# zhuduowang/Change3D

Hardware: AMD Instinct MI355X
Metric: train images/sec (256x256 pairs, X3D-L BCD) (higher is better)
Workload: dtype bf16; 1 GPU; BCD X3D-L bf16, B=32/GPU, 256x256 synthetic LEVIR-CD-shaped pairs, T=3, train step (fwd+BCE/Dice+bwd+Adam); global_batch=32, parallelism=dp1, dist_world_size=1, hip_graph=False, full=False, settle_steps=40, input=resident in HBM

## Files before the change

### change3d_amd/_lib.py

```python
import ctypes as C
import os

_HERE = os.path.dirname(os.path.abspath(__file__))
LIB_PATH = os.environ.get("C3D_LIB") or os.path.join(_HERE, "lib", "libchange3d_hip.so")

DT_F32, DT_BF16 = 0, 1
PRO_NONE, PRO_BN_SE_SWISH, PRO_AFFINE2 = 0, 1, 2
EPI_STORE, EPI_STATS, EPI_SWISH_SE_BWD, EPI_ADD = 0, 1, 2, 3
AUG_NONE, AUG_BCD, AUG_SCD, AUG_BDA = 0, 1, 2, 3
ROWS_DENSE, ROWS_FRAME, ROWS_STRIDE2, ROWS_S2SHIFT = 0, 1, 2, 3
SC_NONE, SC_IDENTITY, SC_BN, SC_RAW = 0, 1, 2, 3
STAT_STRIPES = 16
OPT_SIDE_STREAM, OPT_STEM_MFMA, OPT_CONVT_MFMA, OPT_FUSE_WGRAD, OPT_FOLD_SE, OPT_MASK_IN_DGRAD, OPT_DW_RING, OPT_PW_WGRAD_V2, OPT_DW_FWD_HV, OPT_PW_CFWD, OPT_PW_CDG, OPT_DW_T4 = 0, 1, 2, 3, 4, 5, 6, 7, 8, 9, 10, 11
STAGE_SEPARATE_FINALIZE, STAGE_NO_WEIGHT_IMAGES, STAGE_SEPARATE_RESIDUAL, STAGE_SEPARATE_WGRAD = 1, 2, 4, 8

vp, i32, i64, f32, f64 = C.c_void_p, C.c_int32, C.c_int64, C.c_float, C.c_double


class BnFin(C.Structure):
    _fields_ = [("ticket", vp), ("gamma", vp), ("beta", vp), ("running_mean", vp), ("running_var", vp), ("nbt", vp),
                ("ss", vp), ("mr", vp), ("count", f64), ("momentum", f32), ("eps", f32), ("training", i32),
                ("batch", i32), ("sums", vp)]


class PwArgs(C.Structure):
    _fields_ = [("x", vp), ("x2", vp), ("y", vp), ("e1", vp), ("w", vp), ("pro_p", vp), ("pro_gate", vp),
                ("epi_p", vp), ("epi_gate", vp), ("epi_q", vp), ("stats", vp),
                ("M", i64), ("gstride", i64), ("rows_per_sample", i64),
# ... 85 lines not shown
    "c3d_block_out_fwd_fin": (i32, [vp, C.POINTER(BnFin), vp, C.POINTER(BnFin), i32, vp, i64, i32, i32, i32, vp]),
    "c3d_block_out_bwd": (i32, [vp, vp, vp, vp, vp, vp, vp, vp, vp, i64, i32, i32, i32, vp]),
    "c3d_block_out_bwd_fin": (i32, [vp, vp, vp, vp, vp, vp, vp, vp, vp, i64, i32, i32, i32, C.POINTER(BnFin),
                                    C.POINTER(BnFin), vp]),
    "c3d_frame_absdiff": (i32, [vp, vp, i32, i32, i64, i32, i32, i32, i32, vp]),
    "c3d_enhance_apply": (i32, [vp, vp, vp, i32, i32, i64, i32, i32, i32, vp]),
    "c3d_enhance_bwd_mask": (i32, [vp, vp, vp, i32, i32, i64, i32, i32, i32, vp]),
    "c3d_enhance_bwd_apply": (i32, [vp, vp, vp, vp, i32, i32, i64, i32, i32, i32, i32, vp]),
    "c3d_stem_enhance_fwd": (i32, [vp, vp, vp, vp, i32, i32, i64, i32, i32, i32, i32, i32, vp]),
    "c3d_stem_enhance_mid": (i32, [vp, vp, vp, vp, i32, i32, i64, i32, i32, i32, vp]),
    "c3d_stem_enhance_bwd": (i32, [vp, vp, vp, vp, vp, vp, vp, i32, i32, i64, i32, i32, i32, i32, i32, vp]),
    "c3d_frame_scatter": (i32, [vp, vp, i32, i32, i64, i32, i32, i32, i32, vp]),
    "c3d_stem_fwd": (i32, [vp, vp, vp, vp, vp, i32, i32, i32, i32, i32, vp]),
    "c3d_stem_bwd_dv": (i32, [vp, vp, vp, vp, vp, vp, vp, vp, i32, i32, i32, i32, i32, vp]),
    "c3d_stem_bwd_wx": (i32, [vp, vp, vp, vp, vp, i32, i32, i32, i32, i32, i32, i32, i32, vp]),
    "c3d_convT4s2_fwd": (i32, [vp, vp, vp, vp, i64, vp, i32, i32, i32, i32, i32, vp]),
    "c3d_convT4s2_bwd_data": (i32, [vp, vp, vp, i32, i32, i32, i32, i32, vp]),
    "c3d_convT4s2_wgrad_ws_floats": (i64, [i32, i32, i32, i32]),
    "c3d_convT4s2_wgrad": (i32, [vp, vp, vp, vp, i32, i32, i32, i32, i32, vp]),
    "c3d_col_sum": (i32, [vp, vp, i64, i32, i32, i32, vp]),
    "c3d_head3x3_fwd": (i32, [vp, vp, vp, i32, i32, i32, i32, i32, i32, i32, vp]),
    "c3d_head3x3_bwd_ws_floats": (i64, [i32, i32, i32, i32]),
    "c3d_head3x3_bwd": (i32, [vp, vp, vp, vp, vp, vp, vp, i32, i32, i32, i32, i32, i32, i32, vp]),
    "c3d_bce_dice_fwd": (i32, [vp, vp, i64, vp, vp, vp]),
    "c3d_bce_dice_bwd": (i32, [vp, vp, vp, vp, i64, vp, vp]),
    "c3d_ce2d_fwd": (i32, [vp, vp, i64, i32, i64, i64, i64, i64, vp, vp, vp]),
    "c3d_ce2d_bwd": (i32, [vp, vp, vp, vp, i64, i32, i64, i64, i64, i64, vp, vp]),
    "c3d_cossim_fwd": (i32, [vp, vp, vp, i64, i32, i64, i64, i64, i64, i64, vp, vp, vp]),
    "c3d_cossim_bwd": (i32, [vp, vp, vp, vp, i64, i32, i64, i64, i64, i64, i64, vp, vp, vp]),
    "c3d_adam_step": (i32, [vp, vp, vp, vp, i64, vp, f32, f32, f32, f32, f32, f32, f32, vp]),
# ... 95 lines not shown
```

### change3d_amd/csrc/launch_hints.h

```cpp
#pragma once
#include <cstdint>
#include <hip/hip_runtime.h>
#include "../../include/change3d_hip.h"

extern thread_local int c3d_side_launch;

extern int c3d_option_stem_mfma;
extern int c3d_option_convt_mfma;
extern int c3d_option_dw_ring;
extern int c3d_option_pw_wgrad_v2;
extern int c3d_option_dw_fwd_hv;
extern int c3d_option_pw_cfwd;
extern int c3d_option_pw_cdg;
extern int c3d_option_dw_t4;
#pragma GCC visibility push(hidden)
extern int c3d_option_side_stream;
extern int c3d_option_fuse_wgrad;
extern int c3d_option_fold_se;
extern int c3d_option_mask_in_dgrad;
extern int c3d_option_wgrad_chain;
#pragma GCC visibility pop
bool c3d_detail_pw_cdg_a_shape(int Kp, int Np, int64_t M);
bool c3d_detail_pw_cdg_c_shape(int Kp, int Np, int64_t M, int64_t rows_per_sample);
bool c3d_detail_pw_cdg_a_accepts(const c3d_pw_args* args);
bool c3d_detail_pw_cdg_c_accepts(const c3d_pw_args* args);
int c3d_detail_pw_cdg_a(const c3d_pw_args* args, int* parts_out, void* stream);
int c3d_detail_pw_cdg_c(const c3d_pw_args* args, int* parts_out, void* stream);
int c3d_detail_pw_wgrad_reduce(const float* ws, float* dw, int N, int K, int parts, int sn, int sk, hipStream_t stream);
void c3d_detail_pw_wgrad_v2_forget(const float* ws);
// ... 1 lines not shown
```

### change3d_amd/csrc/options.hip

```cpp
#include "../../include/change3d_hip.h"
#include "common.h"
#include "launch_hints.h"
#include <cstring>
#include <cxxabi.h>

namespace {
enum Norm {
  BOOL,
  CLAMP,
  MASK,
  BIT_OFF,
};
}

#define C3D_OPTIONS(X)                                                    \
  X(C3D_OPT_SIDE_STREAM, c3d_option_side_stream, BOOL, 0, 1)              \
  X(C3D_OPT_STEM_MFMA, c3d_option_stem_mfma, CLAMP, 2, 2)                 \
  X(C3D_OPT_CONVT_MFMA, c3d_option_convt_mfma, BOOL, 0, 1)                \
  X(C3D_OPT_FUSE_WGRAD, c3d_option_fuse_wgrad, MASK, 3, 3)                \
  X(C3D_OPT_FOLD_SE, c3d_option_fold_se, BOOL, 0, 1)                      \
  X(C3D_OPT_MASK_IN_DGRAD, c3d_option_mask_in_dgrad, MASK, 3, 3)          \
  X(C3D_OPT_DW_RING, c3d_option_dw_ring, MASK, 15, 13)                    \
  X(C3D_OPT_PW_WGRAD_V2, c3d_option_pw_wgrad_v2, MASK, 1, 1)              \
  X(C3D_OPT_PW_WGRAD_V2, c3d_option_wgrad_chain, BIT_OFF, 2, 1)           \
  X(C3D_OPT_DW_FWD_HV, c3d_option_dw_fwd_hv, MASK, 7, 5)                  \
  X(C3D_OPT_PW_CFWD, c3d_option_pw_cfwd, MASK, 3, 3)                      \
  X(C3D_OPT_PW_CDG, c3d_option_pw_cdg, MASK, 3, 3)                        \
  X(C3D_OPT_DW_T4, c3d_option_dw_t4, BOOL, 0, 1)

#define X(id, var, how, arg, dflt) int var = dflt;
C3D_OPTIONS(X)
#undef X

extern "C" int c3d_set_option(int32_t option, int32_t value) {
  static const struct { int32_t id; int* var; Norm how; int arg; } rows[] = {
#define X(id, var, how, arg, dflt) {id, &var, how, arg},
      C3D_OPTIONS(X)
#undef X
  };
  int rc = C3D_E_BADARG;
  for (const auto& r : rows) {
    if (r.id != option) continue;
    switch (r.how) {
// ... 35 lines not shown
```

### change3d_amd/csrc/stem.hip

```cpp
#include "common.h"
#include "stem_mfma.h"
#include <cstdlib>
#include "../../include/change3d_hip.h"

namespace {

constexpr int ST_C = 24;
constexpr int ST_CI = 3;
constexpr int ST_TH = 8, ST_TW = 16;
constexpr int ST_MAXT = 5;

template <typename T> struct RawS;
template <> struct RawS<bf16_t> {
  typedef uint4 type;
  static __device__ __forceinline__ type load(const bf16_t* p) { return *reinterpret_cast<const uint4*>(p); }
  static __device__ __forceinline__ void cvt(const type& v, float (&f)[8]) {
    f[0] = __uint_as_float(v.x << 16); f[1] = __uint_as_float(v.x & 0xffff0000u);
    f[2] = __uint_as_float(v.y << 16); f[3] = __uint_as_float(v.y & 0xffff0000u);
    f[4] = __uint_as_float(v.z << 16); f[5] = __uint_as_float(v.z & 0xffff0000u);
    f[6] = __uint_as_float(v.w << 16); f[7] = __uint_as_float(v.w & 0xffff0000u);
  }
};
template <> struct RawS<float> {
  struct type { float4 a, b; };
// ... 449 lines not shown
  const int ntiles = ((W + ST_TW - 1) / ST_TW) * ((H + ST_TH - 1) / ST_TH);
  int bsplit = (2 * 256 + ntiles - 1) / ntiles;
  if (bsplit > B) bsplit = B;
  if (bsplit < 1) bsplit = 1;
  const int tpw = 1;
  dim3 grid(ntiles, bsplit);
  hipStream_t s = reinterpret_cast<hipStream_t>(stream);
  if (dtype == C3D_DT_F32)
    return c3d_launch_lds<stem_bwd_wx_kernel<float>>(grid, SW_THREADS, lds, s, x, w_t, (const float*)dv, dw_t, dP, g, t_first,
                                                     n_frames, per_sample, tpw);
  if (dtype == C3D_DT_BF16)
    return c3d_launch_lds<stem_bwd_wx_kernel<bf16_t>>(grid, SW_THREADS, lds, s, x, w_t, (const bf16_t*)dv, dw_t, dP, g, t_first,
                                                      n_frames, per_sample, tpw);
  return C3D_E_BADARG;
}
```

### change3d_amd/csrc/stem_mfma.h

```cpp
#pragma once
#include <hip/hip_runtime.h>

bool c3d_stem_mfma_enabled();
int c3d_stem_fwd_mfma(const float* x, const float* w_t, const float* w_xy, void* u, double* sums, int B, int T, int H,
                      int W, int dtype, hipStream_t s);
int c3d_stem_bwd_dv_mfma(const float* x, const float* w_t, const float* w_xy, const void* g0, const void* u,
                         const float* coef, void* dv, float* dw_xy, int B, int T, int H, int W, int dtype, hipStream_t s);
int c3d_stem_bwd_wx_mfma(const float* x, const float* w_t, const void* dv, float* dw_t, float* dP, int B, int T, int H,
                         int W, int t_first, int n_frames, int per_sample, int dtype, hipStream_t s);
```

### change3d_amd/csrc/stem_mfma.hip

```cpp
#include "common.h"
#include "stem_mfma.h"
#include "launch_hints.h"
#include <cstdlib>
#include "../../include/change3d_hip.h"

namespace {

constexpr int SC = 24, SCI = 3;
constexpr int TH = 8, TW = 32;
constexpr int IH = TH + 2, IW = TW + 2;
constexpr int IHW = IH * IW;
constexpr int NTHR = 256;
constexpr int KS = 7;

struct Geom { int B, T, H, W; };

__device__ __forceinline__ f32x4_t mfma4(float a, float b, f32x4_t c) {
  return __builtin_amdgcn_mfma_f32_16x16x4f32(a, b, c, 0, 0, 0);
}

template <int TT> struct XTile {
  static constexpr int ITEMS = SCI * TT * IHW;
  static constexpr int NL = (ITEMS + NTHR - 1) / NTHR;
  float r[NL];
// ... 627 lines not shown
      if (tap < 9 && ci < SCI) {
#pragma unroll
        for (int i = 0; i < 4; ++i) wred[(wave * 32 + mt * 16 + 4 * g4 + i) * 32 + ci * 9 + tap] = dwacc[mt][nt][i];
      }
    }
  __syncthreads();
  for (int i = tid; i < SC * 27; i += NTHR) {
    const int c = i / 27, k = i - c * 27;
    float a = 0.f;
#pragma unroll
    for (int w = 0; w < 4; ++w) a += wred[(w * 32 + c) * 32 + k];
    atomicAdd(dw_t + (size_t)c * 27 + k, a);
  }
}

template <typename T, int TT>
int fwd_t(const float* x, const float* w_t, const float* w_xy, void* u, double* sums, const Geom& g, hipStream_t s) {
  const size_t lds = (2 * 4 * 2 * 32 + (size_t)SCI * TT * IHW) * sizeof(float);
  const int ntiles = ((g.W + TW - 1) / TW) * ((g.H + TH - 1) / TH);
  static const int env_tpw = c3d_env("C3D_STEM_FWD_TPW") ? atoi(c3d_env("C3D_STEM_FWD_TPW")) : 0;
  int tpw = 8;
  while (tpw > 1 && (long)((ntiles + tpw - 1) / tpw) * g.B < 1024) tpw >>= 1;
  if (env_tpw > 0) tpw = env_tpw;
  dim3 grid((ntiles + tpw - 1) / tpw, g.B);
  stem_fwd_mfma_kernel<T, TT><<<grid, NTHR, lds, s>>>(x, w_t, w_xy, reinterpret_cast<T*>(u), sums, g, tpw);
  return 0;
}

template <typename T, int TT>
int dv_t(const float* x, const float* w_t, const float* w_xy, const void* g0, const void* u, const float* coef, void* dv,
// ... 21 lines not shown
  if (lds > 160 * 1024) return C3D_E_UNSUPPORTED;
  const int ntiles = ((g.W + TW - 1) / TW) * ((g.H + TH - 1) / TH);
  int bsplit = (2 * 256 + ntiles - 1) / ntiles;
  if (bsplit > g.B) bsplit = g.B;
  if (bsplit < 1) bsplit = 1;
  if (sizeof(T) == 2 && c3d_option_stem_mfma >= 2 && (!dP || n_frames <= (TT - 2 > 0 ? TT - 2 : 1))) {
    size_t lb = ((size_t)TT * IHW * SC + 8 + (size_t)TT * IHW * 4 + 8) * sizeof(bf16_t);
    if (lb < 4 * 32 * 32 * sizeof(float)) lb = 4 * 32 * 32 * sizeof(float);
    return c3d_launch_lds<stem_bwd_wx_bf16_kernel<TT>>(dim3(ntiles, bsplit), NTHR, lb, s, x, w_t, reinterpret_cast<const bf16_t*>(dv),
                                                       dw_t, dP, g, t_first, n_frames, per_sample);
  }
  return c3d_launch_lds<stem_bwd_wx_mfma_kernel<T, TT>>(dim3(ntiles, bsplit), NTHR, lds, s, x, w_t, reinterpret_cast<const T*>(dv),
                                                        dw_t, dP, g, t_first, n_frames, per_sample);
}

#define STEM_DISPATCH(FN, ...)                                                         \
  if (dtype == C3D_DT_F32) {                                                           \
    if (T == 3) return FN<float, 3>(__VA_ARGS__);                                      \
    if (T == 4) return FN<float, 4>(__VA_ARGS__);                                      \
    if (T == 5) return FN<float, 5>(__VA_ARGS__);                                      \
  } else if (dtype == C3D_DT_BF16) {                                                   \
    if (T == 3) return FN<bf16_t, 3>(__VA_ARGS__);                                     \
    if (T == 4) return FN<bf16_t, 4>(__VA_ARGS__);                                     \
    if (T == 5) return FN<bf16_t, 5>(__VA_ARGS__);                                     \
  }                                                                                    \
  return C3D_E_UNSUPPORTED;

}

bool c3d_stem_mfma_enabled() { return c3d_option_stem_mfma != 0; }
// ... 3 lines not shown
  const Geom g{B, T, H, W};
  STEM_DISPATCH(fwd_t, x, w_t, w_xy, u, sums, g, s)
}

int c3d_stem_bwd_dv_mfma(const float* x, const float* w_t, const float* w_xy, const void* g0, const void* u,
                         const float* coef, void* dv, float* dw_xy, int B, int T, int H, int W, int dtype, hipStream_t s) {
  const Geom g{B, T, H, W};
  STEM_DISPATCH(dv_t, x, w_t, w_xy, g0, u, coef, dv, dw_xy, g, s)
}

int c3d_stem_bwd_wx_mfma(const float* x, const float* w_t, const void* dv, float* dw_t, float* dP, int B, int T, int H,
                         int W, int t_first, int n_frames, int per_sample, int dtype, hipStream_t s) {
  const Geom g{B, T, H, W};
  STEM_DISPATCH(wx_t, x, w_t, dv, dw_t, dP, g, t_first, n_frames, per_sample, s)
}
```

### change3d_amd/model/x3d.py

```python
import math

import os

import torch
import torch.nn as nn

from .. import ops
from ..ops import cpad

BN_EPS, BN_MOM = 1e-5, 0.1


def round_width(width, multiplier, min_width=8, divisor=8, ceil=False):
    if not multiplier:
        return width
    width *= multiplier
    min_width = min_width or divisor
    if ceil:
        out = max(min_width, int(math.ceil(width / divisor)) * divisor)
    else:
        out = max(min_width, int(width + divisor / 2) // divisor * divisor)
    if out < 0.9 * width:
        out += divisor
    return int(out)
# ... 56 lines not shown
    g = torch.empty_like(u)
    dsums = torch.zeros(2 * C, dtype=torch.float64, device=dev)
    ops.block_out_bwd(dyc, y, u, None, g, mr, None, dsums, None, M, C, dt)
    return _stem_backward_convs(ctx, xin, u, mr, g, dsums, frames_grad)


def _stem_backward_convs(ctx, xin, u, mr, g, dsums, frames_grad=None):
    stem = ctx.stem
    B, _, T, H, W = xin.shape
    dev, dt = xin.device, ops.dt_code(stem.act_dtype)
    conv_s, conv_t = stem.conv.conv_t, stem.conv.conv_xy
    C = conv_s.weight.shape[0]
    M = B * T * H * W
    coef = _f32(3 * cpad(C), dev)
    ops.bn_bwd_coef(dsums, M, stem.norm, mr, C, coef)
    dv = torch.empty_like(u)
    ops.stem_bwd_dv(xin, conv_s.weight, conv_t.weight, g, u, coef, dv, ops.grad_of(conv_t.weight), B, T, H, W, dt)
    dx = None
    if frames_grad is not None:
        gp, t0, nf = frames_grad
        ops.stem_bwd_wx(xin, conv_s.weight, dv, ops.grad_of(conv_s.weight), gp, B, T, H, W, t0, nf, False, dt)
    elif ctx.x_needs_grad:
        t0, nf = stem.grad_frames if stem.grad_frames is not None else (0, T)
        dx = torch.zeros_like(xin)
        ops.stem_bwd_wx(xin, conv_s.weight, dv, ops.grad_of(conv_s.weight), dx, B, T, H, W, t0, nf, True, dt)
    else:
        ops.stem_bwd_wx(xin, conv_s.weight, dv, ops.grad_of(conv_s.weight), None, B, T, H, W, 0, 0, False, dt)
    return dx


def _assemble_clip(ctx, pre, post, frames):
    ops.require_gpu(pre, "encoder input")
    B, Ci, H, W = pre.shape
    K = frames.shape[2]
    if Ci != 3 or tuple(frames.shape) != (1, 3, K, H, W) or tuple(post.shape) != tuple(pre.shape):
        raise NotImplementedError("clip assembly expects (B,3,H,W) images and (1,3,K,H,W) perception frames")
    clip = torch.empty((B, 3, K + 2, H, W), dtype=torch.float32, device=pre.device)
    ops.build_clip(pre.detach().contiguous().float(), post.detach().contiguous().float(),
                   frames.detach().contiguous().float(), clip, B, K, H, W)
    ctx.frames, ctx.K, ctx.x_needs_grad = frames, K, False
    ctx.need_frames = ctx.needs_input_grad[2]
    return clip

# ... 355 lines not shown
```

### change3d_amd/ops.py

```python
import ctypes as C

import os

import torch

from . import _lib as L
from ._lib import (OPT_CONVT_MFMA, OPT_DW_FWD_HV, OPT_DW_RING, OPT_DW_T4, OPT_FOLD_SE, OPT_FUSE_WGRAD, OPT_MASK_IN_DGRAD, OPT_PW_CDG, OPT_PW_CFWD, OPT_PW_WGRAD_V2, OPT_SIDE_STREAM, OPT_STEM_MFMA, STAGE_NO_WEIGHT_IMAGES, STAGE_SEPARATE_FINALIZE,
                   STAGE_SEPARATE_RESIDUAL, STAGE_SEPARATE_WGRAD)
from ._lib import (DT_BF16, DT_F32, EPI_ADD, EPI_STATS, EPI_STORE, EPI_SWISH_SE_BWD, PRO_AFFINE2,
                   PRO_BN_SE_SWISH, PRO_NONE, ROWS_DENSE, ROWS_FRAME, ROWS_S2SHIFT, ROWS_STRIDE2, SC_BN,
                   SC_IDENTITY, SC_NONE, SC_RAW, STAT_STRIPES)


def cpad(c):
    return (c + 7) // 8 * 8


def dt_code(dtype):
    if dtype == torch.float32:
        return DT_F32
    if dtype == torch.bfloat16:
        return DT_BF16
    raise TypeError(f"unsupported activation dtype {dtype} (float32 | bfloat16)")

# ... 76 lines not shown

def weights_version():
    return _weights_version[0]


def bump_weights_version():
    _weights_version[0] += 1


SIDE_STREAM = os.environ.get("C3D_WGRAD_SIDE", "1") != "0"
_side_streams = {}
_side_pending = []
_side_state = {"seq": 0}


def set_option(option, value):
    L.check(L.lib().c3d_set_option(int(option), int(value)), "c3d_set_option")


def last_kernel():
    return L.lib().c3d_last_kernel().decode()


def launch_count():
    return int(L.lib().c3d_launch_count())


def side_run(fn, *tensors):
    in_backward = False
    if SIDE_STREAM:
        try:
            torch.autograd.Variable._execution_engine.queue_callback(side_join)
# ... 303 lines not shown
            t_dst, 1 if accumulate else 0, dtype, _stream())


def stem_fwd(x, w_t, w_xy, u, sums, B, T, H, W, dtype):
    _launch("c3d_stem_fwd", x.numel() * 4 + u.numel() * _es(dtype), L.lib().c3d_stem_fwd, _p(x), _p(w_t), _p(w_xy), _p(u), _p(sums), B, T, H, W, dtype, _stream())


def stem_bwd_dv(x, w_t, w_xy, g0, u, coef, dv, dw_xy, B, T, H, W, dtype):
    _launch("c3d_stem_bwd_dv", x.numel() * 4 + 3 * u.numel() * _es(dtype), L.lib().c3d_stem_bwd_dv, _p(x), _p(w_t), _p(w_xy), _p(g0), _p(u), _p(coef), _p(dv), _p(dw_xy), B, T, H,
                                    W, dtype, _stream())


def stem_bwd_wx(x, w_t, dv, dw_t, dP, B, T, H, W, t_first, n_frames, per_sample, dtype):
    _launch("c3d_stem_bwd_wx", x.numel() * 4 + dv.numel() * _es(dtype), L.lib().c3d_stem_bwd_wx, _p(x), _p(w_t), _p(dv), _p(dw_t), _p(dP), B, T, H, W, t_first, n_frames,
                                    1 if per_sample else 0, dtype, _stream())


def convT_fwd(inp, w, bias, skip_ptr, skip_bstride, out, B, h, wd, C_, dtype):
    _launch("c3d_convT4s2_fwd", (inp.numel() + 2 * out.numel()) * _es(dtype), L.lib().c3d_convT4s2_fwd, _p(inp), _p(w), _p(bias), skip_ptr, skip_bstride, _p(out), B, h, wd, C_,
                                     dtype, _stream())


def convT_bwd_data(dout, w, din, B, h, wd, C_, dtype):
    _launch("c3d_convT4s2_bwd_data", (dout.numel() + din.numel()) * _es(dtype), L.lib().c3d_convT4s2_bwd_data, _p(dout), _p(w), _p(din), B, h, wd, C_, dtype, _stream())


CONVT_MFMA = os.environ.get("C3D_CONVT_MFMA", "1") != "0"


def convT_wgrad(t, dout, dw, B, h, wd, C_, dtype):
# ... 373 lines not shown
```

### include/change3d_hip.h

```cpp
#ifndef CHANGE3D_HIP_H
#define CHANGE3D_HIP_H
#include <stdint.h>

#ifdef __cplusplus
extern "C" {
#endif

#define C3D_DT_F32 0
#define C3D_DT_BF16 1

#define C3D_E_BADARG (-1)
#define C3D_E_UNSUPPORTED (-2)

int c3d_abi_version(void);
const char* c3d_build_info(void);
int c3d_device_cus(void);

#define C3D_PRO_NONE 0
#define C3D_PRO_BN_SE_SWISH 1
#define C3D_PRO_AFFINE2 2

#define C3D_EPI_STORE 0
#define C3D_EPI_STATS 1
#define C3D_STAT_STRIPES 16
// ... 161 lines not shown
                         int32_t Cp, int32_t t_mid, int32_t dtype, void* stream);
int c3d_stem_enhance_bwd(const void* dout, const void* u, const float* ss, const void* dd, const float* mr, void* g,
                         double* dsums, int32_t B, int32_t T, int64_t HW, int32_t C, int32_t Cp, int32_t t_pre,
                         int32_t t_post, int32_t dtype, void* stream);
int c3d_frame_scatter(const void* src, void* dst, int32_t B, int32_t T, int64_t HW, int32_t Cp,
                      int32_t t_dst, int32_t accumulate, int32_t dtype, void* stream);

int c3d_stem_fwd(const float* x, const float* w_t, const float* w_xy, void* u, double* sums, int32_t B,
                 int32_t T, int32_t H, int32_t W, int32_t dtype, void* stream);
int c3d_stem_bwd_dv(const float* x, const float* w_t, const float* w_xy, const void* g0, const void* u,
                    const float* coef, void* dv, float* dw_xy, int32_t B, int32_t T, int32_t H, int32_t W,
                    int32_t dtype, void* stream);
int c3d_stem_bwd_wx(const float* x, const float* w_t, const void* dv, float* dw_t, float* dP, int32_t B,
                    int32_t T, int32_t H, int32_t W, int32_t t_first, int32_t n_frames, int32_t per_sample,
                    int32_t dtype, void* stream);

int c3d_convT4s2_fwd(const void* in, const float* w, const float* bias, const void* skip,
                     int64_t skip_bstride, void* out, int32_t B, int32_t h, int32_t wd, int32_t C,
                     int32_t dtype, void* stream);
int c3d_convT4s2_bwd_data(const void* dout, const float* w, void* din, int32_t B, int32_t h, int32_t wd,
                          int32_t C, int32_t dtype, void* stream);
int64_t c3d_convT4s2_wgrad_ws_floats(int32_t B, int32_t h, int32_t wd, int32_t C);
int c3d_convT4s2_wgrad(const void* t, const void* dout, float* dw, float* ws, int32_t B, int32_t h, int32_t wd,
                       int32_t C, int32_t dtype, void* stream);
int c3d_col_sum(const void* x, float* out, int64_t M, int32_t C, int32_t Cp, int32_t dtype, void* stream);
int c3d_head3x3_fwd(const void* x, const float* w, float* out, int32_t B, int32_t H, int32_t W, int32_t C,
                    int32_t NC, int32_t has_sigmoid, int32_t dtype, void* stream);
int64_t c3d_head3x3_bwd_ws_floats(int32_t B, int32_t H, int32_t W, int32_t NC);
int c3d_head3x3_bwd(const float* dout, const float* prob, const void* x, const float* w, void* dx,
                    float* dw, float* ws, int32_t B, int32_t H, int32_t W, int32_t C, int32_t NC, int32_t has_sigmoid,
// ... 84 lines not shown
  int32_t dtype;
  int32_t training;
  int32_t flags;
  float momentum, eps;
  const c3d_block_desc* blocks;
} c3d_stage_desc;

int c3d_stage_ws_bytes(const c3d_stage_desc* d, int64_t* ws_fwd_bytes, int64_t* ws_bwd_bytes, int64_t* y_bytes,
                       int64_t* dx_bytes);
int c3d_stage_fwd(const c3d_stage_desc* d, const void* x, void* ws_fwd, void* y, void* stream);
int c3d_stage_bwd(const c3d_stage_desc* d, const void* x, const void* y, const void* dy, void* ws_fwd, void* ws_bwd,
                  void* dx, void* stream);
int c3d_side_join(void* stream);
enum { C3D_OPT_SIDE_STREAM = 0, C3D_OPT_STEM_MFMA = 1, C3D_OPT_CONVT_MFMA = 2, C3D_OPT_FUSE_WGRAD = 3, C3D_OPT_FOLD_SE = 4,
       C3D_OPT_MASK_IN_DGRAD = 5, C3D_OPT_DW_RING = 6, C3D_OPT_PW_WGRAD_V2 = 7, C3D_OPT_DW_FWD_HV = 8, C3D_OPT_PW_CFWD = 9,
       C3D_OPT_PW_CDG = 10, C3D_OPT_DW_T4 = 11 };
int c3d_set_option(int32_t option, int32_t value);
typedef struct c3d_prof_row {
  char name[64];
  int32_t launches, reserved;
  float ms_total, reserved2;
  double bytes_total;
} c3d_prof_row;
int c3d_prof_begin(int32_t flags);
int c3d_prof_end(c3d_prof_row* rows, int32_t cap, int32_t* n_rows);
int c3d_stage_fold_bytes(const c3d_stage_desc* d, int64_t* fold_bytes, int64_t* ws_eval_bytes);
int c3d_stage_fold_bn(const c3d_stage_desc* d, void* fold, void* stream);
int c3d_stage_fwd_folded(const c3d_stage_desc* d, const void* fold, const void* x, void* ws, void* y, void* stream);
int c3d_stage_saved(const c3d_stage_desc* d, int32_t blk, const char* name, int64_t* offset, int64_t* bytes);
const char* c3d_last_kernel(void);
int64_t c3d_launch_count(void);
// ... 59 lines not shown
```

Measured before the change: 1636 images/s.

## Fuse stem backward dv and weight-grad kernels, write only needed frame grads

Adds a fused bf16 MFMA kernel for the X3D stem backward. In one pass it computes the temporal-conv input gradient and both the depthwise temporal and spatial weight gradients, and it stores dv only for the frames whose pixel gradient is needed. A separate kernel then computes the input-pixel gradient from that compact dv. This removes the full-size dv round trip through HBM and a reread of x in the old dv + wx path. In exchange it adds LDS-heavy kernels, an extra launch, and atomic weight-gradient reductions. The path is on by default for T=3 bf16 when at most T-2 frames need gradients.

```diff
diff --git a/change3d_amd/_lib.py b/change3d_amd/_lib.py
--- a/change3d_amd/_lib.py
+++ b/change3d_amd/_lib.py
@@ -11,7 +11,7 @@
 ROWS_DENSE, ROWS_FRAME, ROWS_STRIDE2, ROWS_S2SHIFT = 0, 1, 2, 3
 SC_NONE, SC_IDENTITY, SC_BN, SC_RAW = 0, 1, 2, 3
 STAT_STRIPES = 16
-OPT_SIDE_STREAM, OPT_STEM_MFMA, OPT_CONVT_MFMA, OPT_FUSE_WGRAD, OPT_FOLD_SE, OPT_MASK_IN_DGRAD, OPT_DW_RING, OPT_PW_WGRAD_V2, OPT_DW_FWD_HV, OPT_PW_CFWD, OPT_PW_CDG, OPT_DW_T4 = 0, 1, 2, 3, 4, 5, 6, 7, 8, 9, 10, 11
+OPT_SIDE_STREAM, OPT_STEM_MFMA, OPT_CONVT_MFMA, OPT_FUSE_WGRAD, OPT_FOLD_SE, OPT_MASK_IN_DGRAD, OPT_DW_RING, OPT_PW_WGRAD_V2, OPT_DW_FWD_HV, OPT_PW_CFWD, OPT_PW_CDG, OPT_DW_T4, OPT_STEM_BWD = 0, 1, 2, 3, 4, 5, 6, 7, 8, 9, 10, 11, 13
 STAGE_SEPARATE_FINALIZE, STAGE_NO_WEIGHT_IMAGES, STAGE_SEPARATE_RESIDUAL, STAGE_SEPARATE_WGRAD = 1, 2, 4, 8
 
 vp, i32, i64, f32, f64 = C.c_void_p, C.c_int32, C.c_int64, C.c_float, C.c_double
@@ -127,6 +127,8 @@
     "c3d_stem_fwd": (i32, [vp, vp, vp, vp, vp, i32, i32, i32, i32, i32, vp]),
     "c3d_stem_bwd_dv": (i32, [vp, vp, vp, vp, vp, vp, vp, vp, i32, i32, i32, i32, i32, vp]),
     "c3d_stem_bwd_wx": (i32, [vp, vp, vp, vp, vp, i32, i32, i32, i32, i32, i32, i32, i32, vp]),
+    "c3d_stem_bwd_dv_dw": (i32, [vp, vp, vp, vp, vp, vp, vp, vp, vp, i32, i32, i32, i32, i32, i32, i32, vp]),
+    "c3d_stem_bwd_dp": (i32, [vp, vp, vp, i32, i32, i32, i32, i32, i32, i32, i32, vp]),
     "c3d_convT4s2_fwd": (i32, [vp, vp, vp, vp, i64, vp, i32, i32, i32, i32, i32, vp]),
     "c3d_convT4s2_bwd_data": (i32, [vp, vp, vp, i32, i32, i32, i32, i32, vp]),
     "c3d_convT4s2_wgrad_ws_floats": (i64, [i32, i32, i32, i32]),
diff --git a/change3d_amd/csrc/launch_hints.h b/change3d_amd/csrc/launch_hints.h
--- a/change3d_amd/csrc/launch_hints.h
+++ b/change3d_amd/csrc/launch_hints.h
@@ -13,6 +13,7 @@
 extern int c3d_option_pw_cfwd;
 extern int c3d_option_pw_cdg;
 extern int c3d_option_dw_t4;
+extern int c3d_option_stem_bwd;
 #pragma GCC visibility push(hidden)
 extern int c3d_option_side_stream;
 extern int c3d_option_fuse_wgrad;
diff --git a/change3d_amd/csrc/options.hip b/change3d_amd/csrc/options.hip
--- a/change3d_amd/csrc/options.hip
+++ b/change3d_amd/csrc/options.hip
@@ -26,7 +26,8 @@
   X(C3D_OPT_DW_FWD_HV, c3d_option_dw_fwd_hv, MASK, 7, 5)                  \
   X(C3D_OPT_PW_CFWD, c3d_option_pw_cfwd, MASK, 3, 3)                      \
   X(C3D_OPT_PW_CDG, c3d_option_pw_cdg, MASK, 3, 3)                        \
-  X(C3D_OPT_DW_T4, c3d_option_dw_t4, BOOL, 0, 1)
+  X(C3D_OPT_DW_T4, c3d_option_dw_t4, BOOL, 0, 1)                          \
+  X(C3D_OPT_STEM_BWD, c3d_option_stem_bwd, MASK, 1, 1)
 
 #define X(id, var, how, arg, dflt) int var = dflt;
 C3D_OPTIONS(X)
diff --git a/change3d_amd/csrc/stem.hip b/change3d_amd/csrc/stem.hip
--- a/change3d_amd/csrc/stem.hip
+++ b/change3d_amd/csrc/stem.hip
@@ -487,3 +487,20 @@
                                                       n_frames, per_sample, tpw);
   return C3D_E_BADARG;
 }
+
+extern "C" int c3d_stem_bwd_dv_dw(const float* x, const float* w_t, const float* w_xy, const void* g0, const void* u,
+                                  const float* coef, void* dvc, float* dw_xy, float* dw_t, int32_t B, int32_t T, int32_t H,
+                                  int32_t W, int32_t t_first, int32_t n_frames, int32_t dtype, void* stream) {
+  if (!x || !w_t || !w_xy || !g0 || !u || !coef || !dw_xy || !dw_t || B <= 0 || T <= 0 || T > ST_MAXT || H <= 0 || W <= 0)
+    return C3D_E_BADARG;
+  if (n_frames < 0 || t_first < 0 || t_first + n_frames > T || (n_frames > 0 && !dvc)) return C3D_E_BADARG;
+  return c3d_stem_bwd_dvw_mfma(x, w_t, w_xy, g0, u, coef, dvc, dw_xy, dw_t, B, T, H, W, t_first, n_frames, dtype,
+                               reinterpret_cast<hipStream_t>(stream));
+}
+
+extern "C" int c3d_stem_bwd_dp(const float* w_t, const void* dvc, float* dP, int32_t B, int32_t T, int32_t H, int32_t W,
+                               int32_t t_first, int32_t n_frames, int32_t per_sample, int32_t dtype, void* stream) {
+  if (!w_t || !dvc || !dP || B <= 0 || T <= 0 || T > ST_MAXT || H <= 0 || W <= 0) return C3D_E_BADARG;
+  if (t_first < 0 || n_frames <= 0 || t_first + n_frames > T) return C3D_E_BADARG;
+  return c3d_stem_bwd_dp_mfma(w_t, dvc, dP, B, T, H, W, t_first, n_frames, per_sample, dtype, reinterpret_cast<hipStream_t>(stream));
+}
diff --git a/change3d_amd/csrc/stem_mfma.h b/change3d_amd/csrc/stem_mfma.h
--- a/change3d_amd/csrc/stem_mfma.h
+++ b/change3d_amd/csrc/stem_mfma.h
@@ -8,3 +8,8 @@
                          const float* coef, void* dv, float* dw_xy, int B, int T, int H, int W, int dtype, hipStream_t s);
 int c3d_stem_bwd_wx_mfma(const float* x, const float* w_t, const void* dv, float* dw_t, float* dP, int B, int T, int H,
                          int W, int t_first, int n_frames, int per_sample, int dtype, hipStream_t s);
+int c3d_stem_bwd_dvw_mfma(const float* x, const float* w_t, const float* w_xy, const void* g0, const void* u, const float* coef,
+                          void* dvc, float* dw_xy, float* dw_t, int B, int T, int H, int W, int t_first, int n_frames, int dtype,
+                          hipStream_t s);
+int c3d_stem_bwd_dp_mfma(const float* w_t, const void* dvc, float* dP, int B, int T, int H, int W, int t_first, int n_frames,
+                         int per_sample, int dtype, hipStream_t s);
diff --git a/change3d_amd/csrc/stem_mfma.hip b/change3d_amd/csrc/stem_mfma.hip
--- a/change3d_amd/csrc/stem_mfma.hip
+++ b/change3d_amd/csrc/stem_mfma.hip
@@ -665,6 +665,305 @@
   }
 }
 
+template <int TT>
+__global__ __launch_bounds__(NTHR, TT == 3 ? 2 : 1) void stem_bwd_dp_bf16_kernel(
+    const float* __restrict__ w_t, const bf16_t* __restrict__ dvc, float* __restrict__ dP, const Geom g, const int t_first,
+    const int n_frames, const int per_sample) {
+  constexpr int NF = TT - 2 > 0 ? TT - 2 : 1;
+  extern __shared__ __attribute__((aligned(16))) float sm[];
+  bf16_t* dt_ = reinterpret_cast<bf16_t*>(sm);
+  bf16_t* zs = dt_ + (size_t)TT * IHW * SC;
+  const int tid = threadIdx.x, lane = tid & 63, wave = tid >> 6;
+  const int g4 = lane >> 4, li = lane & 15;
+  const int tiles_x = (g.W + TW - 1) / TW;
+  if (tid < 2) *reinterpret_cast<uint2*>(zs + (size_t)tid * 4) = make_uint2(0, 0);
+  uint4 wA[9];
+#pragma unroll
+  for (int sp = 0; sp < 9; ++sp) {
+    float f[8];
+#pragma unroll
+    for (int j = 0; j < 8; ++j) {
+      const int c = 8 * g4 + j;
+      f[j] = (li < SCI && c < SC) ? w_t[c * 27 + li * 9 + sp] : 0.f;
+    }
+    wA[sp] = make_uint4(pack_bf16x2(f[0], f[1]), pack_bf16x2(f[2], f[3]), pack_bf16x2(f[4], f[5]), pack_bf16x2(f[6], f[7]));
+  }
+  f32x4_t dxa[NF][4];
+#pragma unroll
+  for (int k = 0; k < NF; ++k)
+#pragma unroll
+    for (int q = 0; q < 4; ++q) dxa[k][q] = f32x4_t{0.f, 0.f, 0.f, 0.f};
+  const int tl = blockIdx.x;
+  const int tx = tl % tiles_x, ty = tl / tiles_x;
+  const int y0 = ty * TH, x0 = tx * TW;
+  for (int b = blockIdx.y; b < g.B; b += gridDim.y) {
+    constexpr int DITEMS = NF * IHW * 3, DNL = (DITEMS + NTHR - 1) / NTHR;
+    uint4 dr[DNL];
+#pragma unroll
+    for (int j = 0; j < DNL; ++j) {
+      const int i = tid + j * NTHR;
+      const int cvv = i % 3;
+      int q = i / 3;
+      const int ix = q % IW;
+      q /= IW;
+      const int iy = q % IH, k = q / IH;
+      const int gy = y0 - 1 + iy, gx = x0 - 1 + ix;
+      dr[j] = make_uint4(0, 0, 0, 0);
+      if (i < DITEMS && k < n_frames && gy >= 0 && gy < g.H && gx >= 0 && gx < g.W)
+        dr[j] = *reinterpret_cast<const uint4*>(dvc + ((((size_t)b * n_frames + k) * g.H + gy) * g.W + gx) * SC + cvv * 8);
+    }
+    __syncthreads();
+#pragma unroll
+    for (int j = 0; j < DNL; ++j) {
+      const int i = tid + j * NTHR;
+      if (i < DITEMS) *reinterpret_cast<uint4*>(dt_ + (size_t)i * 8) = dr[j];
+    }
+    __syncthreads();
+#pragma unroll
+    for (int k = 0; k < NF; ++k) {
+      if (k < n_frames) {
+        const int t = t_first + k;
+#pragma unroll
+        for (int q = 0; q < 4; ++q) {
+          const int r = 2 * wave + (q >> 1), xs = (q & 1) * 16;
+          f32x4_t acc = per_sample ? f32x4_t{0.f, 0.f, 0.f, 0.f} : dxa[k][q];
+#pragma unroll
+          for (int sp = 0; sp < 9; ++sp) {
+            const int ky = sp / 3, kx = sp - ky * 3;
+            const bf16_t* bp = g4 < 3 ? dt_ + ((size_t)(k * IH + r + 2 - ky) * IW + xs + li + 2 - kx) * SC + 8 * g4 : zs;
+            acc = mfma32b(wA[sp], *reinterpret_cast<const uint4*>(bp), acc);
+          }
+          if (per_sample) {
+            const int gy = y0 + r, gx = x0 + xs + li;
+            if (g4 == 0 && gy < g.H && gx < g.W) {
+#pragma unroll
+              for (int ci = 0; ci < SCI; ++ci) dP[((((size_t)b * SCI + ci) * TT + t) * g.H + gy) * g.W + gx] = acc[ci];
+            }
+          } else {
+            dxa[k][q] = acc;
+          }
+        }
+      }
+    }
+  }
+  if (!per_sample) {
+#pragma unroll
+    for (int k = 0; k < NF; ++k) {
+      if (k < n_frames) {
+#pragma unroll
+        for (int q = 0; q < 4; ++q) {
+          const int gy = y0 + 2 * wave + (q >> 1), gx = x0 + (q & 1) * 16 + li;
+          if (g4 == 0 && gy < g.H && gx < g.W) {
+#pragma unroll
+            for (int ci = 0; ci < SCI; ++ci) {
+              float* dst = dP + (((size_t)ci * n_frames + k) * g.H + gy) * g.W + gx;
+              if (gridDim.y == 1) *dst += dxa[k][q][ci];
+              else atomicAdd(dst, dxa[k][q][ci]);
+            }
+          }
+        }
+      }
+    }
+  }
+}
+
+constexpr int DVL = 3 * 16 * SC + 8;
+constexpr int XBN = 3 * IHW * 4;
+
+__global__ __launch_bounds__(NTHR) void stem_bwd_dvw_bf16_kernel(
+    const float* __restrict__ x, const float* __restrict__ w_t, const float* __restrict__ w_xy,
+    const bf16_t* __restrict__ g0, const bf16_t* __restrict__ u, const float* __restrict__ coef, bf16_t* __restrict__ dvc,
+    float* __restrict__ dw_xy, float* __restrict__ dw_t, const Geom g, const int t_first, const int n_frames,
+    const int tiles_per_wg) {
+  constexpr int TT = 3;
+  typedef bf16_t T;
+  extern __shared__ __attribute__((aligned(16))) float sm[];
+  float* red = sm;
+  float* xt = red + 4 * 5 * 32;
+  bf16_t* xb = reinterpret_cast<bf16_t*>(xt + SCI * TT * IHW);
+  bf16_t* dvl = xb + (size_t)2 * XBN;
+  const int tid = threadIdx.x, lane = tid & 63, wave = tid >> 6;
+  const int kk = lane >> 4, n = lane & 15;
+  const int tiles_x = (g.W + TW - 1) / TW, tiles_y = (g.H + TH - 1) / TH;
+  const int ntiles = tiles_x * tiles_y;
+  const int b = blockIdx.y;
+  for (int i = tid; i < 2 * TT * IHW; i += NTHR) *reinterpret_cast<uint2*>(xb + (size_t)i * 4) = make_uint2(0, 0);
+  bf16_t* dw_ = dvl + wave * DVL;
+  if (lane < 4) *reinterpret_cast<uint32_t*>(dw_ + 3 * 16 * SC + 2 * lane) = 0u;
+  SpatialFrag sf;
+  sf.init(w_t, lane, TT);
+  float wx[5][2][4], cA[2][4], cB[2][4], cC[2][4], dwx[5][2][4];
+#pragma unroll
+  for (int mt = 0; mt < 2; ++mt)
+#pragma unroll
+    for (int i = 0; i < 4; ++i) {
+      const int ch = mt * 16 + 4 * kk + i;
+      const bool ok = ch < SC;
+      cA[mt][i] = ok ? coef[ch] : 0.f; cB[mt][i] = ok ? coef[SC + ch] : 0.f; cC[mt][i] = ok ? coef[2 * SC + ch] : 0.f;
+#pragma unroll
+      for (int dt = 0; dt < 5; ++dt) { wx[dt][mt][i] = ok ? w_xy[ch * 5 + dt] : 0.f; dwx[dt][mt][i] = 0.f; }
+    }
+  const int pxl = 4 * kk + (n >> 2);
+  int boff[3];
+#pragma unroll
+  for (int nt = 0; nt < 3; ++nt) {
+    int tap = 4 * nt + (n & 3);
+    if (tap > 8) tap = 8;
+    boff[nt] = ((tap / 3) * IW + pxl + tap % 3) * 4;
+  }
+  const int aoff = pxl * SC + 4 * (n & 3);
+  f32x4_t dwacc[2][3];
+#pragma unroll
+  for (int mt = 0; mt < 2; ++mt)
+#pragma unroll
+    for (int nt = 0; nt < 3; ++nt) dwacc[mt][nt] = f32x4_t{0.f, 0.f, 0.f, 0.f};
+
+  auto dw_step = [&](const bf16_t* xrow) {
+    s16x4_t af[TT][2], bf[TT][3];
+#pragma unroll
+    for (int t = 0; t < TT; ++t) {
+      const bf16_t* ap = dw_ + t * 16 * SC + aoff;
+      af[t][0] = __builtin_amdgcn_ds_read_tr16_b64_v4i16((lds_s16x4_ptr_t)ap);
+      af[t][1] = __builtin_amdgcn_ds_read_tr16_b64_v4i16((lds_s16x4_ptr_t)(ap + 16));
+#pragma unroll
+      for (int nt = 0; nt < 3; ++nt)
+        bf[t][nt] = __builtin_amdgcn_ds_read_tr16_b64_v4i16((lds_s16x4_ptr_t)(xrow + (size_t)t * IHW * 4 + boff[nt]));
+    }
+#pragma unroll
+    for (int t = 0; t < TT; ++t)
+#pragma unroll
+      for (int nt = 0; nt < 3; ++nt) {
+        dwacc[0][nt] = __builtin_amdgcn_mfma_f32_16x16x16bf16_1k(af[t][0], bf[t][nt], dwacc[0][nt], 0, 0, 0);
+        dwacc[1][nt] = __builtin_amdgcn_mfma_f32_16x16x16bf16_1k(af[t][1], bf[t][nt], dwacc[1][nt], 0, 0, 0);
+      }
+    __builtin_amdgcn_fence(__ATOMIC_ACQUIRE, "wavefront");
+    __builtin_amdgcn_wave_barrier();
+  };
+  const bf16_t* pend = nullptr;
+
+  const int tl0 = blockIdx.x * tiles_per_wg;
+  const int tl1 = tl0 + tiles_per_wg < ntiles ? tl0 + tiles_per_wg : ntiles;
+  XTile<TT> xq;
+  if (tl0 < tl1) xq.issue(x, g, b, (tl0 / tiles_x) * TH, (tl0 % tiles_x) * TW, tid);
+  for (int tl = tl0; tl < tl1; ++tl) {
+    const int tx = tl % tiles_x, ty = tl / tiles_x;
+    bf16_t* xbt = xb + (size_t)(tl & 1) * XBN;
+    __syncthreads();
+    xq.commit(xt, tid);
+#pragma unroll
+    for (int j = 0; j < XTile<TT>::NL; ++j) {
+      const int i = tid + j * NTHR;
+      if (i < XTile<TT>::ITEMS) {
+        const int q = i / IHW, p = i - q * IHW;
+        const int ci = q / TT, t = q - ci * TT;
+        xbt[(size_t)(t * IHW + p) * 4 + ci] = f32_to_bf16(xq.r[j]);
+      }
+    }
+    __syncthreads();
+    if (tl + 1 < tl1) xq.issue(x, g, b, ((tl + 1) / tiles_x) * TH, ((tl + 1) % tiles_x) * TW, tid);
+#pragma unroll 1
+    for (int rp = 0; rp < 4; ++rp) {
+      const int row = 2 * wave + (rp >> 1), pt = rp & 1;
+      const int gy = ty * TH + row, gx = tx * TW + pt * 16 + n;
+      const bool in_img = gy < g.H && gx < g.W;
+      Q4<T>::raw gr[TT][2], ur[TT][2];
+#pragma unroll
+      for (int t = 0; t < TT; ++t)
+#pragma unroll
+        for (int mt = 0; mt < 2; ++mt) {
+          gr[t][mt] = make_uint2(0, 0); ur[t][mt] = make_uint2(0, 0);
+          if (in_img && mt * 16 + 4 * kk < SC) {
+            const size_t off = ((((size_t)b * TT + t) * g.H + gy) * g.W + gx) * SC + mt * 16 + 4 * kk;
+            gr[t][mt] = Q4<T>::load(g0 + off);
+            ur[t][mt] = Q4<T>::load(u + off);
+          }
+        }
+      f32x4_t v[TT][2];
+      sf.conv<TT>(v, xt, row, pt, n);
+      if (pend) dw_step(pend);
+      pend = xbt + (size_t)(row * IW + pt * 16) * 4;
+#pragma unroll
+      for (int mt = 0; mt < 2; ++mt) {
+        if (mt * 16 + 4 * kk >= SC) continue;
+        float du[TT][4];
+#pragma unroll
+        for (int t = 0; t < TT; ++t) {
+          float gg[4], uu[4];
+          Q4<T>::cvt(gr[t][mt], gg);
+          Q4<T>::cvt(ur[t][mt], uu);
+#pragma unroll
+          for (int i = 0; i < 4; ++i) du[t][i] = in_img ? fmaf(cA[mt][i], gg[i], fmaf(cC[mt][i], uu[i], cB[mt][i])) : 0.f;
+        }
+#pragma unroll
+        for (int t = 0; t < TT; ++t) {
+          float o[4] = {0.f, 0.f, 0.f, 0.f};
+#pragma unroll
+          for (int dt = 0; dt < 5; ++dt) {
+            const int to = t - dt + 2;
+            if (to >= 0 && to < TT) {
+#pragma unroll
+              for (int i = 0; i < 4; ++i) o[i] = fmaf(wx[dt][mt][i], du[to][i], o[i]);
+            }
+            const int ti = t + dt - 2;
+            if (ti >= 0 && ti < TT) {
+#pragma unroll
+              for (int i = 0; i < 4; ++i) dwx[dt][mt][i] = fmaf(du[t][i], v[ti][mt][i], dwx[dt][mt][i]);
+            }
+          }
+          uint2 ob;
+          ob.x = pack_bf16x2(o[0], o[1]); ob.y = pack_bf16x2(o[2], o[3]);
+          *reinterpret_cast<uint2*>(dw_ + (t * 16 + n) * SC + mt * 16 + 4 * kk) = ob;
+          if (in_img && t >= t_first && t < t_first + n_frames)
+            *reinterpret_cast<uint2*>(dvc + ((((size_t)b * n_frames + (t - t_first)) * g.H + gy) * g.W + gx) * SC + mt * 16 + 4 * kk) = ob;
+        }
+      }
+      __builtin_amdgcn_fence(__ATOMIC_RELEASE, "wavefront");
+      __builtin_amdgcn_wave_barrier();
+    }
+  }
+  if (pend) dw_step(pend);
+  __syncthreads();
+  float* wred = xt;
+#pragma unroll
+  for (int dt = 0; dt < 5; ++dt)
+#pragma unroll
+    for (int mt = 0; mt < 2; ++mt)
+#pragma unroll
+      for (int i = 0; i < 4; ++i) {
+        const float r = row16_sum(dwx[dt][mt][i]);
+        if (n == 0) red[(wave * 5 + dt) * 32 + mt * 16 + 4 * kk + i] = r;
+      }
+#pragma unroll
+  for (int mt = 0; mt < 2; ++mt)
+#pragma unroll
+    for (int nt = 0; nt < 3; ++nt) {
+      const int tap = 4 * nt + (n >> 2), ci = n & 3;
+      if (tap < 9 && ci < SCI) {
+#pragma unroll
+        for (int i = 0; i < 4; ++i) wred[(wave * 32 + mt * 16 + 4 * kk + i) * 32 + ci * 9 + tap] = dwacc[mt][nt][i];
+      }
+    }
+  __syncthreads();
+  for (int i = tid; i < 5 * SC; i += NTHR) {
+    const int dt = i / SC, c = i - dt * SC;
+    float a = 0.f;
+#pragma unroll
+    for (int w = 0; w < 4; ++w) a += red[(w * 5 + dt) * 32 + c];
+    atomicAdd(dw_xy + c * 5 + dt, a);
+  }
+  for (int i = tid; i < SC * 27; i += NTHR) {
+    const int c = i / 27, k = i - c * 27;
+    float a = 0.f;
+#pragma unroll
+    for (int w = 0; w < 4; ++w) a += wred[(w * 32 + c) * 32 + k];
+    atomicAdd(dw_t + (size_t)c * 27 + k, a);
+  }
+}
+constexpr size_t DVW_LDS = (4 * 5 * 32 + (size_t)SCI * 3 * IHW) * sizeof(float) + ((size_t)2 * XBN + 4 * DVL) * sizeof(bf16_t);
+static_assert(DVW_LDS >= (4 * 5 * 32 + 4 * 32 * 32) * sizeof(float), "the d w_t reduction tile lies over xt / xb / dvl");
+static_assert((SCI * 3 * IHW * sizeof(float)) % 16 == 0 && (3 * IHW * 4 * sizeof(bf16_t)) % 16 == 0 && (DVL * sizeof(bf16_t)) % 16 == 0,
+              "transposed reads want 8-byte aligned chunks");
+
 template <typename T, int TT>
 int fwd_t(const float* x, const float* w_t, const float* w_xy, void* u, double* sums, const Geom& g, hipStream_t s) {
   const size_t lds = (2 * 4 * 2 * 32 + (size_t)SCI * TT * IHW) * sizeof(float);
@@ -716,6 +1015,29 @@
                                                         dw_t, dP, g, t_first, n_frames, per_sample);
 }
 
+int dvw_launch(const float* x, const float* w_t, const float* w_xy, const void* g0, const void* u, const float* coef, void* dvc,
+               float* dw_xy, float* dw_t, const Geom& g, int t_first, int n_frames, hipStream_t s) {
+  const int ntiles = ((g.W + TW - 1) / TW) * ((g.H + TH - 1) / TH);
+  int tpw = 16;
+  while (tpw > 1 && (long)((ntiles + tpw - 1) / tpw) * g.B < 2L * 256) tpw >>= 1;
+  if (tpw > ntiles) tpw = ntiles;
+  return c3d_launch_lds<stem_bwd_dvw_bf16_kernel>(dim3((ntiles + tpw - 1) / tpw, g.B), NTHR, DVW_LDS, s, x, w_t, w_xy,
+                                                  reinterpret_cast<const bf16_t*>(g0), reinterpret_cast<const bf16_t*>(u), coef,
+                                                  reinterpret_cast<bf16_t*>(dvc), dw_xy, dw_t, g, t_first, n_frames, tpw);
+}
+
+int dp_launch(const float* w_t, const void* dvc, float* dP, const Geom& g, int t_first, int n_frames, int per_sample,
+              hipStream_t s) {
+  constexpr int TT = 3;
+  const int ntiles = ((g.W + TW - 1) / TW) * ((g.H + TH - 1) / TH);
+  int bsplit = (2 * 256 + ntiles - 1) / ntiles;
+  if (bsplit > g.B) bsplit = g.B;
+  if (bsplit < 1) bsplit = 1;
+  const size_t lb = ((size_t)(TT - 2) * IHW * SC + 8) * sizeof(bf16_t);
+  return c3d_launch_lds<stem_bwd_dp_bf16_kernel<TT>>(dim3(ntiles, bsplit), NTHR, lb, s, w_t, reinterpret_cast<const bf16_t*>(dvc), dP,
+                                                     g, t_first, n_frames, per_sample);
+}
+
 #define STEM_DISPATCH(FN, ...)                                                         \
   if (dtype == C3D_DT_F32) {                                                           \
     if (T == 3) return FN<float, 3>(__VA_ARGS__);                                      \
@@ -749,3 +1071,20 @@
   const Geom g{B, T, H, W};
   STEM_DISPATCH(wx_t, x, w_t, dv, dw_t, dP, g, t_first, n_frames, per_sample, s)
 }
+
+static bool c3d_stem_bwd_fused_shape(int T, int n_frames, int dtype) {
+  return c3d_option_stem_mfma >= 2 && (c3d_option_stem_bwd & 1) && T == 3 && dtype == C3D_DT_BF16 && n_frames <= T - 2;
+}
+
+int c3d_stem_bwd_dvw_mfma(const float* x, const float* w_t, const float* w_xy, const void* g0, const void* u, const float* coef,
+                          void* dvc, float* dw_xy, float* dw_t, int B, int T, int H, int W, int t_first, int n_frames, int dtype,
+                          hipStream_t s) {
+  if (!c3d_stem_bwd_fused_shape(T, n_frames, dtype)) return C3D_E_UNSUPPORTED;
+  return dvw_launch(x, w_t, w_xy, g0, u, coef, dvc, dw_xy, dw_t, Geom{B, T, H, W}, t_first, n_frames, s);
+}
+
+int c3d_stem_bwd_dp_mfma(const float* w_t, const void* dvc, float* dP, int B, int T, int H, int W, int t_first, int n_frames,
+                         int per_sample, int dtype, hipStream_t s) {
+  if (!c3d_stem_bwd_fused_shape(T, n_frames, dtype)) return C3D_E_UNSUPPORTED;
+  return dp_launch(w_t, dvc, dP, Geom{B, T, H, W}, t_first, n_frames, per_sample, s);
+}
diff --git a/change3d_amd/model/x3d.py b/change3d_amd/model/x3d.py
--- a/change3d_amd/model/x3d.py
+++ b/change3d_amd/model/x3d.py
@@ -94,6 +94,14 @@
     M = B * T * H * W
     coef = _f32(3 * cpad(C), dev)
     ops.bn_bwd_coef(dsums, M, stem.norm, mr, C, coef)
+    if frames_grad is not None:
+        nf = frames_grad[2]
+    elif ctx.x_needs_grad:
+        nf = stem.grad_frames[1] if stem.grad_frames is not None else T
+    else:
+        nf = 0
+    if ops.stem_bwd_fused(T, nf, dt):
+        return _stem_backward_convs_fused(ctx, xin, u, g, coef, frames_grad)
     dv = torch.empty_like(u)
     ops.stem_bwd_dv(xin, conv_s.weight, conv_t.weight, g, u, coef, dv, ops.grad_of(conv_t.weight), B, T, H, W, dt)
     dx = None
@@ -107,6 +115,27 @@
     else:
         ops.stem_bwd_wx(xin, conv_s.weight, dv, ops.grad_of(conv_s.weight), None, B, T, H, W, 0, 0, False, dt)
     return dx
+
+
+def _stem_backward_convs_fused(ctx, xin, u, g, coef, frames_grad):
+    stem = ctx.stem
+    B, _, T, H, W = xin.shape
+    dt = ops.dt_code(stem.act_dtype)
+    conv_s, conv_t = stem.conv.conv_t, stem.conv.conv_xy
+    C = conv_s.weight.shape[0]
+    if frames_grad is not None:
+        dP, t0, nf = frames_grad
+    elif ctx.x_needs_grad:
+        t0, nf = stem.grad_frames if stem.grad_frames is not None else (0, T)
+        dP = torch.zeros_like(xin)
+    else:
+        dP, t0, nf = None, 0, 0
+    dvc = torch.empty((B, nf, H, W, C), dtype=u.dtype, device=u.device) if nf else None
+    ops.stem_bwd_dv_dw(xin, conv_s.weight, conv_t.weight, g, u, coef, dvc, ops.grad_of(conv_t.weight),
+                       ops.grad_of(conv_s.weight), B, T, H, W, t0, nf, dt)
+    if nf:
+        ops.stem_bwd_dp(conv_s.weight, dvc, dP, B, T, H, W, t0, nf, frames_grad is None, dt)
+    return dP if frames_grad is None else None
 
 
 def _assemble_clip(ctx, pre, post, frames):
diff --git a/change3d_amd/ops.py b/change3d_amd/ops.py
--- a/change3d_amd/ops.py
+++ b/change3d_amd/ops.py
@@ -5,7 +5,7 @@
 import torch
 
 from . import _lib as L
-from ._lib import (OPT_CONVT_MFMA, OPT_DW_FWD_HV, OPT_DW_RING, OPT_DW_T4, OPT_FOLD_SE, OPT_FUSE_WGRAD, OPT_MASK_IN_DGRAD, OPT_PW_CDG, OPT_PW_CFWD, OPT_PW_WGRAD_V2, OPT_SIDE_STREAM, OPT_STEM_MFMA, STAGE_NO_WEIGHT_IMAGES, STAGE_SEPARATE_FINALIZE,
+from ._lib import (OPT_CONVT_MFMA, OPT_DW_FWD_HV, OPT_DW_RING, OPT_DW_T4, OPT_FOLD_SE, OPT_FUSE_WGRAD, OPT_MASK_IN_DGRAD, OPT_PW_CDG, OPT_PW_CFWD, OPT_PW_WGRAD_V2, OPT_SIDE_STREAM, OPT_STEM_BWD, OPT_STEM_MFMA, STAGE_NO_WEIGHT_IMAGES, STAGE_SEPARATE_FINALIZE,
                    STAGE_SEPARATE_RESIDUAL, STAGE_SEPARATE_WGRAD)
 from ._lib import (DT_BF16, DT_F32, EPI_ADD, EPI_STATS, EPI_STORE, EPI_SWISH_SE_BWD, PRO_AFFINE2,
                    PRO_BN_SE_SWISH, PRO_NONE, ROWS_DENSE, ROWS_FRAME, ROWS_S2SHIFT, ROWS_STRIDE2, SC_BN,
@@ -114,8 +114,21 @@
 _side_state = {"seq": 0}
 
 
+STEM_BWD_BITS = 1
+_options = {OPT_STEM_MFMA: 2, OPT_STEM_BWD: 1}
+
+
 def set_option(option, value):
     L.check(L.lib().c3d_set_option(int(option), int(value)), "c3d_set_option")
+    if int(option) == OPT_STEM_BWD:
+        _options[OPT_STEM_BWD] = int(value) & STEM_BWD_BITS
+    elif int(option) == OPT_STEM_MFMA:
+        _options[OPT_STEM_MFMA] = min(max(int(value), 0), 2)
+
+
+def stem_bwd_fused(T, n_frames, dtype):
+    return (bool(_options[OPT_STEM_BWD] & 1) and _options[OPT_STEM_MFMA] >= 2 and T == 3 and dtype == DT_BF16
+            and n_frames <= T - 2)
 
 
 def last_kernel():
@@ -449,6 +462,16 @@
 def stem_bwd_wx(x, w_t, dv, dw_t, dP, B, T, H, W, t_first, n_frames, per_sample, dtype):
     _launch("c3d_stem_bwd_wx", x.numel() * 4 + dv.numel() * _es(dtype), L.lib().c3d_stem_bwd_wx, _p(x), _p(w_t), _p(dv), _p(dw_t), _p(dP), B, T, H, W, t_first, n_frames,
                                     1 if per_sample else 0, dtype, _stream())
+
+
+def stem_bwd_dv_dw(x, w_t, w_xy, g0, u, coef, dvc, dw_xy, dw_t, B, T, H, W, t_first, n_frames, dtype):
+    _launch("c3d_stem_bwd_dv_dw", x.numel() * 4 + (2 * u.numel() + (dvc.numel() if dvc is not None else 0)) * _es(dtype), L.lib().c3d_stem_bwd_dv_dw,
+            _p(x), _p(w_t), _p(w_xy), _p(g0), _p(u), _p(coef), _p(dvc), _p(dw_xy), _p(dw_t), B, T, H, W, t_first, n_frames, dtype, _stream())
+
+
+def stem_bwd_dp(w_t, dvc, dP, B, T, H, W, t_first, n_frames, per_sample, dtype):
+    _launch("c3d_stem_bwd_dp", dvc.numel() * _es(dtype), L.lib().c3d_stem_bwd_dp, _p(w_t), _p(dvc), _p(dP), B, T, H, W, t_first, n_frames,
+            1 if per_sample else 0, dtype, _stream())
 
 
 def convT_fwd(inp, w, bias, skip_ptr, skip_bstride, out, B, h, wd, C_, dtype):
diff --git a/include/change3d_hip.h b/include/change3d_hip.h
--- a/include/change3d_hip.h
+++ b/include/change3d_hip.h
@@ -199,6 +199,11 @@
 int c3d_stem_bwd_wx(const float* x, const float* w_t, const void* dv, float* dw_t, float* dP, int32_t B,
                     int32_t T, int32_t H, int32_t W, int32_t t_first, int32_t n_frames, int32_t per_sample,
                     int32_t dtype, void* stream);
+int c3d_stem_bwd_dv_dw(const float* x, const float* w_t, const float* w_xy, const void* g0, const void* u,
+                       const float* coef, void* dvc, float* dw_xy, float* dw_t, int32_t B, int32_t T, int32_t H, int32_t W,
+                       int32_t t_first, int32_t n_frames, int32_t dtype, void* stream);
+int c3d_stem_bwd_dp(const float* w_t, const void* dvc, float* dP, int32_t B, int32_t T, int32_t H, int32_t W,
+                    int32_t t_first, int32_t n_frames, int32_t per_sample, int32_t dtype, void* stream);
 
 int c3d_convT4s2_fwd(const void* in, const float* w, const float* bias, const void* skip,
                      int64_t skip_bstride, void* out, int32_t B, int32_t h, int32_t wd, int32_t C,
@@ -313,7 +318,7 @@
 int c3d_side_join(void* stream);
 enum { C3D_OPT_SIDE_STREAM = 0, C3D_OPT_STEM_MFMA = 1, C3D_OPT_CONVT_MFMA = 2, C3D_OPT_FUSE_WGRAD = 3, C3D_OPT_FOLD_SE = 4,
        C3D_OPT_MASK_IN_DGRAD = 5, C3D_OPT_DW_RING = 6, C3D_OPT_PW_WGRAD_V2 = 7, C3D_OPT_DW_FWD_HV = 8, C3D_OPT_PW_CFWD = 9,
-       C3D_OPT_PW_CDG = 10, C3D_OPT_DW_T4 = 11 };
+       C3D_OPT_PW_CDG = 10, C3D_OPT_DW_T4 = 11, C3D_OPT_STEM_BWD = 13  };
 int c3d_set_option(int32_t option, int32_t value);
 typedef struct c3d_prof_row {
   char name[64];
```

Result: no change. 1641 images/s, median of 6 (+0.3%).
